# LambdaLabsML/distributed-training-guide

Measured on NVIDIA H100. Metric: tokens/sec (device-timed, max over ranks) Llama-2-7B seq 4096 bf16 training, higher is better.
Workload: dtype bf16; 1 GPU; model=meta-llama/Llama-2-7b-hf, global_batch=1, seq_len=4096, parallelism=dp1 (ddp+zero1), optimizer=AdamW, bf16 parameters and states

## Files before the change

distributed_training_guide_b200/csrc/gemm_common.cuh:

```cuda
#pragma once
#include <cuda.h>
#include <cuda_bf16.h>
#include <cstdint>

#include "common.cuh"

#ifndef DTG_DEFAULT_GEMM_VARIANT
#define DTG_DEFAULT_GEMM_VARIANT 3
#endif

namespace dtg {

template <int CG>
struct GemmCfg {
  static constexpr int THREADS = 384;
  static constexpr int BM = 128;
  static constexpr int BN = 256;
  static constexpr int BK = 64;
  static constexpr int B_ROWS = BN / CG;
  static constexpr int A_BYTES = BM * BK * 2;
  static constexpr int B_BYTES = BN * BK * 2;
  static constexpr int STAGE_BYTES = A_BYTES + B_BYTES;
  static constexpr int STAGES = 4;
  static constexpr int BAR_BYTES = 256;
  static constexpr int SMEM_BYTES = STAGES * STAGE_BYTES + BAR_BYTES + 1024;
  static constexpr int COMM_PIECE = 32768;
  static constexpr int COMM_SLOTS = STAGES * STAGE_BYTES / COMM_PIECE;
  static constexpr int GATHER_PIECE = 16384;
  static constexpr int GATHER_BYTES = 2 * GATHER_PIECE;
  static_assert(2 * STAGES + (COMM_SLOTS > 2 ? COMM_SLOTS : 2) <= BAR_BYTES / 8, "barrier area");
};

template <int N>
struct TmapSet {
  CUtensorMap m[N];
};

struct GemmDist {
  int rows_per_peer;
  int m_tile_shift;
  int k_shift;
  __nv_bfloat16* c_ptr[kMaxRanks];
  const char* ag_src[kMaxRanks];
  uint32_t* ag_flags;
  uint32_t ag_epoch;
  uint32_t* pads[kMaxRanks];
  uint32_t bar_epoch;
  int n_comm;
  int rank, nranks;
  long long tile_bytes;
  const char* bg_src[kMaxRanks];
  char* bg_dst;
  long long bg_per_bytes;
  long long bg_begin, bg_end;
  uint32_t* bg_cnt;
  uint32_t bg_target;
  int bg_chunk_shift;
  int bg_row_bytes;
  int bg_rows;
  int n_tile_shift;
  int group_m, num_n_tiles;
};

#ifdef __CUDACC__
__host__ __device__ __forceinline__ int tile_m(int t, int num_m_tiles, const GemmDist& d) {
  int m = t % num_m_tiles + d.m_tile_shift;
  return m >= num_m_tiles ? m - num_m_tiles : m;
}
__host__ __device__ __forceinline__ void tile_mn(int t, int num_m_tiles, const GemmDist& d, int local_m_tiles, int& m, int& n) {
  if (local_m_tiles <= 0) {
    if (d.group_m > 0 && d.group_m < num_m_tiles) {
      const int per_group = d.group_m * d.num_n_tiles;
      const int g = t / per_group, r = t - g * per_group;
      const int m0 = g * d.group_m;
      const int rest_m = num_m_tiles - m0;
      const int gsz = d.group_m < rest_m ? d.group_m : rest_m;
      m = m0 + r % gsz;
      n = r / gsz;
      return;
    }
    m = tile_m(t, num_m_tiles, d);
    n = t / num_m_tiles + d.n_tile_shift;
    if (n >= d.num_n_tiles && d.n_tile_shift) n -= d.num_n_tiles;
    return;
  }
  const int num_n = d.k_shift;
  const int phase_a = local_m_tiles * num_n;
  int mm;
  if (t < phase_a) {
    mm = t % local_m_tiles;
    n = t / local_m_tiles;
  } else {
    const int u = t - phase_a, rest = num_m_tiles - local_m_tiles;
    mm = local_m_tiles + u % rest;
    n = u / rest;
  }
  mm += d.m_tile_shift;
  m = mm >= num_m_tiles ? mm - num_m_tiles : mm;
}
#endif

CUtensorMap make_tmap_bf16(const void* base, int rank, const uint64_t* dims, const uint64_t* strides_bytes,
                           const uint32_t* box, bool swizzle128);
CUtensorMap make_tmap_2d(const void* base, uint64_t inner, uint64_t outer, uint64_t row_stride_bytes,
                         uint32_t box_inner, uint32_t box_outer);
void set_gemm_variant(int v);
int default_gemm_variant();

}
```

distributed_training_guide_b200/csrc/gemm_wgmma.cu:

```cuda
#include <cuda.h>
#include <cudaTypedefs.h>

#include <cstdlib>
#include <mutex>
#include <unordered_map>

#include "api.h"
#include "common.cuh"
#include "gemm_common.cuh"
#include "ptx.cuh"

namespace dtg {

using namespace ptx;

__device__ __forceinline__ long long bg_clamp(const GemmDist& d, long long x) {
  return x < d.bg_begin ? d.bg_begin : (x > d.bg_end ? d.bg_end : x);
}
__device__ __forceinline__ int bg_rotation_chunks(const GemmDist& d) {
  return (int)((bg_clamp(d, (long long)(d.rank + 1) * d.bg_per_bytes) - d.bg_begin) >> d.bg_chunk_shift);
}

template <bool A_K, bool B_K, int CG, int A_MODE = 0, int B_MODE = 0, int C_MODE = 0, int ET = 0>
__global__ void __launch_bounds__(GemmCfg<CG>::THREADS, 1)
gemm_bf16_kernel(const __grid_constant__ TmapSet<(A_MODE ? kMaxRanks : 1)> tmAs,
                 const __grid_constant__ TmapSet<(B_MODE ? kMaxRanks : 1)> tmBs, const __grid_constant__ GemmDist dist,
                 __nv_bfloat16* __restrict__ C, int M, int N, int K, long long ldc, int accumulate, int num_m_tiles,
                 int num_tiles, const float* __restrict__ scale_a, const float* __restrict__ scale_b) {
  static_assert(ET == 0 || (A_K && B_K && A_MODE == 0 && B_MODE == 0 && C_MODE == 0),
                "the fp8 GEMM takes K-major operands from one tensor map each");
  using Cfg = GemmCfg<CG>;
  constexpr int BK = ET ? 2 * Cfg::BK : Cfg::BK;
  extern __shared__ uint8_t smem_raw[];
  uint8_t* smem = reinterpret_cast<uint8_t*>((reinterpret_cast<uintptr_t>(smem_raw) + 1023) & ~uintptr_t(1023));
  uint64_t* bars = reinterpret_cast<uint64_t*>(smem + Cfg::STAGES * Cfg::STAGE_BYTES);
  uint64_t* full = bars;
  uint64_t* empty = bars + Cfg::STAGES;
  uint64_t* comm_bar = bars + 2 * Cfg::STAGES;

  const int warp = threadIdx.x >> 5;
  const int lane = threadIdx.x & 31;
  const uint32_t cta_rank = (CG == 2) ? cluster_ctarank() : 0u;
  const int n_comm = (A_MODE == 3) ? dist.n_comm : 0;
  const bool is_comm = (A_MODE == 3) && (int)(blockIdx.x / CG) < n_comm;
  const int cluster_id = (int)(blockIdx.x / CG) - n_comm;
  const int num_clusters = (int)(gridDim.x / CG) - n_comm;
  const int num_kb = (K + BK - 1) / BK;
  const int local_m_tiles = (A_MODE == 3) ? dist.rows_per_peer / (Cfg::BM * CG) : 0;

  if (threadIdx.x == 0) {
    prefetch_tensormap(&tmAs.m[0]);
    prefetch_tensormap(&tmBs.m[0]);
    for (int i = 0; i < Cfg::STAGES; ++i) {
      mbar_init(&full[i], 1);
      mbar_init(&empty[i], 2 * CG);
    }
    if constexpr (A_MODE == 3)
      for (int i = 0; i < Cfg::COMM_SLOTS; ++i) mbar_init(&comm_bar[i], 1);
    if constexpr (B_MODE == 3)
      for (int i = 0; i < 2; ++i) mbar_init(&comm_bar[i], 1);
    fence_barrier_init();
  }
  if (CG == 2) cluster_sync(); else __syncthreads();

  if (is_comm) {
    if (warp == 0 && elect_one()) {
      const int cidx = (int)blockIdx.x;
      const int ncta = n_comm * CG;
      const int t_ = dist.nranks, rk = dist.rank;
      for (int p = 0; p < t_; ++p) st_release_sys(dist.pads[p] + cidx * kMaxRanks + rk, dist.bar_epoch);
      for (int p = 0; p < t_; ++p) {
        const uint32_t* mine = dist.pads[rk] + cidx * kMaxRanks + p;
        const unsigned long long t0 = global_timer_ns();
        while ((int32_t)(ld_acquire_sys(mine) - dist.bar_epoch) < 0)
          if (global_timer_ns() - t0 > kWaitTimeoutNs)
            __trap();
      }
      constexpr uint32_t PIECE = Cfg::COMM_PIECE;
      constexpr int NB = Cfg::COMM_SLOTS, AHEAD = NB - 2;
      const int lmt = local_m_tiles > 0 ? local_m_tiles : 1;
      const int remote_tiles = (t_ - 1) * lmt;
      const uint32_t pieces_per_tile = (uint32_t)(dist.tile_bytes / PIECE);
      uint32_t issued = 0, stored = 0;
      for (int r = cidx; r < remote_tiles; r += ncta) {
        const int k = 1 + r / lmt, within = r % lmt;
        const int owner = (rk + k) % t_;
        const int m_tile = owner * lmt + within;
        const char* src = dist.ag_src[k] + (long long)m_tile * dist.tile_bytes;
        char* dst = const_cast<char*>(dist.ag_src[0]) + (long long)m_tile * dist.tile_bytes;
        uint32_t li = 0;
        for (uint32_t si = 0; si < pieces_per_tile; ++si) {
          while (li < pieces_per_tile && li < si + AHEAD) {
            const uint32_t slot = issued % NB;
            bulk_wait_group_read<1>();
            mbar_arrive_expect_tx(&comm_bar[slot], PIECE);
            bulk_load_g2s(smem + slot * PIECE, src + (long long)li * PIECE, PIECE, &comm_bar[slot]);
            ++issued;
            ++li;
          }
          const uint32_t slot = stored % NB;
          mbar_wait_mma(&comm_bar[slot], (stored / NB) & 1);
          bulk_store_s2g(dst + (long long)si * PIECE, smem + slot * PIECE, PIECE);
          bulk_commit_group();
          ++stored;
        }
        bulk_wait_group<0>();
        fence_proxy_async_all();
        st_release_gpu(dist.ag_flags + m_tile, dist.ag_epoch);
      }
    }
  } else if (warp == 0) {
    if (elect_one()) {
      int stage = 0;
      uint32_t phase = 0;
      [[maybe_unused]] int bg_wm = 0;
      [[maybe_unused]] const int bg_nch = (B_MODE == 3) ? (int)((dist.bg_end - dist.bg_begin) >> dist.bg_chunk_shift) : 0;
      [[maybe_unused]] const int bg_rot = (B_MODE == 3) ? bg_rotation_chunks(dist) : 0;
      [[maybe_unused]] const int bg_my0 = (B_MODE == 3)
          ? (int)((bg_clamp(dist, (long long)dist.rank * dist.bg_per_bytes) - dist.bg_begin) >> dist.bg_chunk_shift) : 0;
      [[maybe_unused]] const int bg_tail = bg_nch - bg_rot;
      [[maybe_unused]] auto bg_wait_rows = [&](int r0, int r1) {
        if (r1 > dist.bg_rows) r1 = dist.bg_rows;
        if (r0 >= r1) return;
        const int c0 = (int)(((long long)r0 * dist.bg_row_bytes) >> dist.bg_chunk_shift);
        const int c1 = (int)((((long long)r1 * dist.bg_row_bytes) - 1) >> dist.bg_chunk_shift);
        int need = 0;
        for (int c = c0; c <= c1; ++c) {
          if (c >= bg_my0 && c < bg_rot) continue;
          const int ci = c >= bg_rot ? c - bg_rot : bg_tail + c;
          need = ci + 1 > need ? ci + 1 : need;
        }
        if (need <= bg_wm) return;
        const uint32_t* cnt = dist.bg_cnt + (dist.bg_begin >> dist.bg_chunk_shift);
        while (bg_wm < need) {
          const int c = bg_wm < bg_tail ? bg_rot + bg_wm : bg_wm - bg_tail;
// ... 71 lines not shown
                tma_load_2d_mc(&tmB, &full[stage], sb + (cta_rank * (Cfg::B_ROWS / 64) + j) * 8192, nb + 64 * j, b_k0,
                               0b11);
            }
          }
          if (++stage == Cfg::STAGES) { stage = 0; phase ^= 1; }
        }
      }
    }
  } else if (warp == 1 && !is_comm) {
    if constexpr (B_MODE == 3) {
      if (elect_one()) {
        constexpr uint32_t PIECE = Cfg::GATHER_PIECE;
        uint8_t* gs = smem + Cfg::STAGES * Cfg::STAGE_BYTES + Cfg::BAR_BYTES;
        const int ch = (int)blockIdx.x, nr = dist.nranks, rk = dist.rank;
        for (int p = 0; p < nr && dist.bar_epoch; ++p)
          st_release_sys(dist.pads[p] + ch * kMaxRanks + rk, dist.bar_epoch);
        for (int p = 0; p < nr && dist.bar_epoch; ++p) {
          const uint32_t* mine = dist.pads[rk] + ch * kMaxRanks + p;
          const unsigned long long t0 = global_timer_ns();
          while ((int32_t)(ld_acquire_sys(mine) - dist.bar_epoch) < 0)
            if (global_timer_ns() - t0 > kWaitTimeoutNs)
              __trap();
        }
        static_assert(PIECE == (1u << 14), "16 KB pieces");
        const long long my_lo = bg_clamp(dist, (long long)rk * dist.bg_per_bytes);
        const long long my_hi = bg_clamp(dist, (long long)(rk + 1) * dist.bg_per_bytes);
        const long long total = (dist.bg_end - dist.bg_begin) / PIECE;
        const long long mine = (my_hi - my_lo) / PIECE;
        const long long np = total - mine;
        const long long after = (dist.bg_end - my_hi) / PIECE;
        uint32_t* const cnt = dist.bg_cnt;
        auto flat_of = [&](long long i) {
          return i < after ? my_hi + i * (long long)PIECE : dist.bg_begin + (i - after) * (long long)PIECE;
        };
        auto issue = [&](long long i, uint32_t it) {
          const long long flat = flat_of(i);
          const int owner = (int)(flat / dist.bg_per_bytes);
          const char* src = dist.bg_src[owner] + (flat - (long long)owner * dist.bg_per_bytes);
          const uint32_t slot = it & 1;
          mbar_arrive_expect_tx(&comm_bar[slot], PIECE);
          bulk_load_g2s(gs + slot * PIECE, src, PIECE, &comm_bar[slot]);
        };
        const long long first = blockIdx.x, stride = gridDim.x;
        uint32_t it = 0;
        long long prev_flat = -1;
        if (first < np) issue(first, 0);
        for (long long i = first; i < np; i += stride, ++it) {
          if (i + stride < np) {
            bulk_wait_group_read<0>();
            issue(i + stride, it + 1);
          }
          const uint32_t slot = it & 1;
          mbar_wait_mma(&comm_bar[slot], (it >> 1) & 1);
          const long long flat = flat_of(i);
          bulk_store_s2g(dist.bg_dst + flat, gs + slot * PIECE, PIECE);
          bulk_commit_group();
          if (prev_flat >= 0) {
            bulk_wait_group<1>();
            fence_proxy_async_all();
            red_release_gpu_add(cnt + (prev_flat >> dist.bg_chunk_shift), 1u);
          }
          prev_flat = flat;
        }
        if (prev_flat >= 0) {
          bulk_wait_group<0>();
          fence_proxy_async_all();
          red_release_gpu_add(cnt + (prev_flat >> dist.bg_chunk_shift), 1u);
        }
      }
    }
  } else if (warp >= 4 && !is_comm) {
    const int half = (warp >> 2) - 1;
    const int wq = warp & 3;
    const bool signal = (threadIdx.x & 127) == 0;
    const uint32_t peer_empty = (CG == 2) ? mapa(smem_u32(&empty[0]), cta_rank ^ 1u) : 0u;
    auto release = [&](int s) {
      if (signal) {
        mbar_arrive(&empty[s]);
        if constexpr (CG == 2) mbar_arrive_cluster(peer_empty + (uint32_t)(s * 8));
      }
    };
    int stage = 0;
    uint32_t phase = 0;
    for (int t = cluster_id; t < num_tiles; t += num_clusters) {
      int tm_, tn_;
      tile_mn(t, num_m_tiles, dist, local_m_tiles, tm_, tn_);
      const int m0 = tm_ * (Cfg::BM * CG) + (int)cta_rank * Cfg::BM + half * 64;
      const int n0 = tn_ * Cfg::BN;
      float acc[128];
#pragma unroll
      for (int i = 0; i < 128; ++i) acc[i] = 0.f;
      int prev = -1;
      for (int kb = 0; kb < num_kb; ++kb) {
        mbar_wait_mma(&full[stage], phase);
        const uint32_t a_base = smem_u32(smem + stage * Cfg::STAGE_BYTES) + (uint32_t)(half * 8192);
        const uint32_t b_base = smem_u32(smem + stage * Cfg::STAGE_BYTES + Cfg::A_BYTES);
        wgmma_fence();
        fence_regs(acc);
        if constexpr (ET == 0) {
#pragma unroll
          for (int k = 0; k < Cfg::BK / 16; ++k) {
            const uint64_t da = A_K ? desc_kmajor_sw128(a_base + k * 32) : desc_mnmajor_sw128(a_base + k * 2048, 8192);
            const uint64_t db = B_K ? desc_kmajor_sw128(b_base + k * 32) : desc_mnmajor_sw128(b_base + k * 2048, 8192);
            wgmma_m64n256k16_ss<A_K ? 0 : 1, B_K ? 0 : 1>(acc, da, db, 1u);
          }
        } else {
#pragma unroll
          for (int k = 0; k < BK / 32; ++k)
            wgmma_m64n256k32_fp8_ss<ET>(acc, desc_kmajor_sw128(a_base + k * 32), desc_kmajor_sw128(b_base + k * 32), 1u);
        }
        wgmma_commit();
        wgmma_wait<1>();
        fence_regs(acc);
        if (prev >= 0) release(prev);
        prev = stage;
        if (++stage == Cfg::STAGES) { stage = 0; phase ^= 1; }
      }
      wgmma_wait<0>();
      fence_regs(acc);
      if (prev >= 0) release(prev);
      [[maybe_unused]] float deq = 1.f;
      if constexpr (ET != 0) deq = scale_a[0] * scale_b[0];
      const int r0 = m0 + wq * 16 + (lane >> 2);
      const int c0 = n0 + 2 * (lane & 3);
#pragma unroll
      for (int h = 0; h < 2; ++h) {
        const int row = r0 + 8 * h;
        if (row >= M) continue;
        __nv_bfloat16* crow = C + (size_t)row * ldc;
        if constexpr (C_MODE == 1) {
          const int owner = row / dist.rows_per_peer;
          crow = dist.c_ptr[owner < kMaxRanks ? owner : 0] + (size_t)(row - owner * dist.rows_per_peer) * ldc;
        }
#pragma unroll
        for (int j = 0; j < 32; ++j) {
          const int col = c0 + 8 * j;
          if (col < N) {
            float x = acc[4 * j + 2 * h], y = acc[4 * j + 2 * h + 1];
            if constexpr (ET != 0) {
              x *= deq;
              y *= deq;
            }
            __nv_bfloat162* p = reinterpret_cast<__nv_bfloat162*>(crow + col);
            if (accumulate) {
              const float2 g = __bfloat1622float2(*p);
              x += g.x;
              y += g.y;
            }
            *p = __floats2bfloat162_rn(x, y);
          }
        }
      }
    }
  }

  if (CG == 2) cluster_sync();
}


static PFN_cuTensorMapEncodeTiled_v12000 get_encode_fn() {
  static PFN_cuTensorMapEncodeTiled_v12000 fn = nullptr;
  if (!fn) {
    void* p = nullptr;
    cudaDriverEntryPointQueryResult qres;
    DTG_CUDA_CHECK(cudaGetDriverEntryPoint("cuTensorMapEncodeTiled", &p, cudaEnableDefault, &qres));
    if (qres != cudaDriverEntryPointSuccess || !p) throw std::runtime_error("cuTensorMapEncodeTiled unavailable");
    fn = reinterpret_cast<PFN_cuTensorMapEncodeTiled_v12000>(p);
  }
  return fn;
}

static CUtensorMap make_tmap_typed(CUtensorMapDataType dtype, const void* base, int rank, const uint64_t* dims,
                                   const uint64_t* strides_bytes, const uint32_t* box, bool swizzle128) {
  static thread_local bool ctx_bound = false;
  if (!ctx_bound) {
    int dev = 0;
    DTG_CUDA_CHECK(cudaGetDevice(&dev));
    DTG_CUDA_CHECK(cudaSetDevice(dev));
    DTG_CUDA_CHECK(cudaFree(nullptr));
    ctx_bound = true;
  }
  CUtensorMap m;
  cuuint64_t gdim[5];
  cuuint64_t gstr[4];
  cuuint32_t bdim[5], estr[5];
  for (int i = 0; i < rank; ++i) {
    gdim[i] = dims[i];
    bdim[i] = box[i];
    estr[i] = 1;
    if (i > 0) gstr[i - 1] = strides_bytes[i - 1];
  }
  CUresult r = get_encode_fn()(&m, dtype, (cuuint32_t)rank, const_cast<void*>(base), gdim,
                               gstr, bdim, estr, CU_TENSOR_MAP_INTERLEAVE_NONE,
                               swizzle128 ? CU_TENSOR_MAP_SWIZZLE_128B : CU_TENSOR_MAP_SWIZZLE_NONE,
                               CU_TENSOR_MAP_L2_PROMOTION_L2_256B, CU_TENSOR_MAP_FLOAT_OOB_FILL_NONE);
  if (r != CUDA_SUCCESS) {
    throw std::runtime_error("cuTensorMapEncodeTiled failed with code " + std::to_string((int)r) +
                             " (base must be 16B aligned, strides multiples of 16B)");
  }
  return m;
}

CUtensorMap make_tmap_bf16(const void* base, int rank, const uint64_t* dims, const uint64_t* strides_bytes,
                           const uint32_t* box, bool swizzle128) {
  return make_tmap_typed(CU_TENSOR_MAP_DATA_TYPE_BFLOAT16, base, rank, dims, strides_bytes, box, swizzle128);
}

CUtensorMap make_tmap_2d(const void* base, uint64_t inner, uint64_t outer, uint64_t row_stride_bytes, uint32_t box_inner,
                         uint32_t box_outer) {
  uint64_t dims[2] = {inner, outer};
  uint64_t strides[1] = {row_stride_bytes};
  uint32_t box[2] = {box_inner, box_outer};
  return make_tmap_bf16(base, 2, dims, strides, box, true);
}

static CUtensorMap make_tmap_2d_u8(const void* base, uint64_t inner, uint64_t outer, uint64_t row_stride_bytes,
                                   uint32_t box_inner, uint32_t box_outer) {
  uint64_t dims[2] = {inner, outer};
  uint64_t strides[1] = {row_stride_bytes};
  uint32_t box[2] = {box_inner, box_outer};
  return make_tmap_typed(CU_TENSOR_MAP_DATA_TYPE_UINT8, base, 2, dims, strides, box, true);
}

static int g_gemm_variant = 0;
void set_gemm_variant(int v) { g_gemm_variant = v; }
int default_gemm_variant() {
  if (g_gemm_variant) return g_gemm_variant;
  static int env = -1;
  if (env < 0) {
    const char* e = getenv("DTG_GEMM_VARIANT");
    env = e ? atoi(e) : DTG_DEFAULT_GEMM_VARIANT;
  }
  return env;
}

template <bool A_K, bool B_K, int CG, int A_MODE, int B_MODE, int C_MODE, int ET = 0>
static void launch_gemm(const void* const* a_srcs, const void* const* b_srcs, void* C, int M, int N, int K,
                        long long lda, long long ldb, long long ldc, bool accumulate, GemmDist dist, int nranks,
                        cudaStream_t s, const float* scale_a = nullptr, const float* scale_b = nullptr) {
  using Cfg = GemmCfg<CG>;
  constexpr int ESIZE = ET ? 1 : 2;
  TmapSet<(A_MODE ? kMaxRanks : 1)> tmA;
  TmapSet<(B_MODE ? kMaxRanks : 1)> tmB;
  const int rpp = dist.rows_per_peer;
  for (int p = 0; p < ((A_MODE == 1 || A_MODE == 2) ? nranks : 1); ++p) {
    const int rows = (A_MODE == 1) ? rpp : M;
    const int ks = (A_MODE == 2) ? rpp : K;
    if constexpr (ET != 0) tmA.m[p] = make_tmap_2d_u8(a_srcs[p], ks, rows, lda, 128, Cfg::BM);
    else tmA.m[p] = A_K ? make_tmap_2d(a_srcs[p], ks, rows, lda * 2, 64, Cfg::BM) : make_tmap_2d(a_srcs[p], rows, ks, lda * 2, 64, 64);
  }
  for (int p = 0; p < ((B_MODE == 1 || B_MODE == 2) ? nranks : 1); ++p) {
    const int ks = (B_MODE == 2) ? rpp : K;
    if constexpr (ET != 0) tmB.m[p] = make_tmap_2d_u8(b_srcs[p], ks, N, ldb, 128, Cfg::B_ROWS);
    else tmB.m[p] = B_K ? make_tmap_2d(b_srcs[p], ks, N, ldb * 2, 64, Cfg::B_ROWS) : make_tmap_2d(b_srcs[p], N, ks, ldb * 2, 64, 64);
  }
  for (int p = ((A_MODE == 1 || A_MODE == 2) ? nranks : 1); p < (A_MODE ? kMaxRanks : 1); ++p) tmA.m[p] = tmA.m[0];
  for (int p = ((B_MODE == 1 || B_MODE == 2) ? nranks : 1); p < (B_MODE ? kMaxRanks : 1); ++p) tmB.m[p] = tmB.m[0];
  const int num_m_tiles = (M + Cfg::BM * CG - 1) / (Cfg::BM * CG);
  const int num_n_tiles = (N + Cfg::BN - 1) / Cfg::BN;
  const int num_tiles = num_m_tiles * num_n_tiles;
  auto kern = gemm_bf16_kernel<A_K, B_K, CG, A_MODE, B_MODE, C_MODE, ET>;
  constexpr int kSmem = Cfg::SMEM_BYTES + (B_MODE == 3 ? Cfg::GATHER_BYTES : 0);
  static bool attr_set = false;
  if (!attr_set) {
    DTG_CUDA_CHECK(cudaFuncSetAttribute(kern, cudaFuncAttributeMaxDynamicSharedMemorySize, kSmem));
    attr_set = true;
  }
  dist.num_n_tiles = num_n_tiles;
  if constexpr (A_MODE == 0 && B_MODE == 0 && C_MODE == 0) {
    static const long long budget = []() {
      const char* e = getenv("DTG_GEMM_L2_BUDGET_MB");
      return (long long)(e ? atoi(e) : 16) << 20;
    }();
    const long long panel = (long long)Cfg::BM * CG * K * ESIZE;
    long long gm = budget / (panel > 0 ? panel : 1);
    if (gm < 8) gm = 8;
    dist.group_m = gm >= num_m_tiles ? 0 : (int)gm;
  }
  int clusters = sm_count() / CG;
  if constexpr (A_MODE == 3) {
    dist.k_shift = num_n_tiles;
    int gemm_clusters = clusters - dist.n_comm;
    if (gemm_clusters > num_tiles) gemm_clusters = num_tiles;
    clusters = gemm_clusters + dist.n_comm;
  } else if (clusters > num_tiles) {
    clusters = num_tiles;
  }
  cudaLaunchConfig_t cfg{};
  cfg.gridDim = dim3(clusters * CG);
  cfg.blockDim = dim3(Cfg::THREADS);
  cfg.dynamicSmemBytes = kSmem;
  cfg.stream = s;
  cudaLaunchAttribute attrs[1];
  attrs[0].id = cudaLaunchAttributeClusterDimension;
  attrs[0].val.clusterDim.x = CG;
  attrs[0].val.clusterDim.y = 1;
  attrs[0].val.clusterDim.z = 1;
  cfg.attrs = attrs;
  cfg.numAttrs = 1;
  DTG_CUDA_CHECK(cudaLaunchKernelEx(&cfg, kern, tmA, tmB, dist, (__nv_bfloat16*)C, M, N, K, ldc, accumulate ? 1 : 0,
                                    num_m_tiles, num_tiles, scale_a, scale_b));
  note_launch();
}

int gemm_max_active_clusters(int cg) {
  cudaLaunchConfig_t cfg{};
  cfg.blockDim = dim3(GemmCfg<1>::THREADS);
  cudaLaunchAttribute attrs[1];
  attrs[0].id = cudaLaunchAttributeClusterDimension;
  attrs[0].val.clusterDim.x = cg;
  attrs[0].val.clusterDim.y = 1;
  attrs[0].val.clusterDim.z = 1;
  cfg.attrs = attrs;
  cfg.numAttrs = 1;
  int n = -1;
  if (cg == 2) {
    auto kern = gemm_bf16_kernel<true, true, 2, 0, 0, 0>;
    cfg.gridDim = dim3(sm_count());
    cfg.dynamicSmemBytes = GemmCfg<2>::SMEM_BYTES;
    cudaFuncSetAttribute(kern, cudaFuncAttributeMaxDynamicSharedMemorySize, GemmCfg<2>::SMEM_BYTES);
    cudaOccupancyMaxActiveClusters(&n, kern, &cfg);
  } else {
    auto kern = gemm_bf16_kernel<true, true, 1, 0, 0, 0>;
    cfg.gridDim = dim3(sm_count());
    cfg.dynamicSmemBytes = GemmCfg<1>::SMEM_BYTES;
    cudaFuncSetAttribute(kern, cudaFuncAttributeMaxDynamicSharedMemorySize, GemmCfg<1>::SMEM_BYTES);
    cudaOccupancyMaxActiveClusters(&n, kern, &cfg);
  }
  return n;
}

static void check_gemm_bases(const char* who, const void* A, const void* B, const void* C) {
  const struct { const void* p; const char* name; } ops[3] = {{A, "A"}, {B, "B"}, {C, "C"}};
  for (const auto& o : ops)
    if (reinterpret_cast<uintptr_t>(o.p) % 16)
      throw std::runtime_error(std::string(who) + ": " + o.name + " must start at a 16-byte aligned address");
}

static void gemm_empty_k(void* C, int M, int N, long long ldc, bool accumulate, cudaStream_t s) {
  if (!accumulate)
    DTG_CUDA_CHECK(cudaMemset2DAsync(C, (size_t)ldc * 2, 0, (size_t)N * 2, (size_t)M, s));
}

void gemm_bf16(const void* A, const void* B, void* C, int M, int N, int K, long long lda, long long ldb, long long ldc,
               bool a_kmajor, bool b_kmajor, bool accumulate, int variant, cudaStream_t s) {
  if (M <= 0 || N <= 0) return;
  if ((N % 8) || (ldc % 8) || (lda % 8) || (ldb % 8))
    throw std::runtime_error("gemm_bf16: N and the leading dimensions must be multiples of 8 elements");
  check_gemm_bases("gemm_bf16", A, B, C);
  if (K <= 0) return gemm_empty_k(C, M, N, ldc, accumulate, s);
  if (variant == 0) variant = default_gemm_variant();
  if (variant == 3) variant = (M > 128) ? 2 : 1;
  const int cg = (variant == 2) ? 2 : 1;
  const void* as[1] = {A};
  const void* bs[1] = {B};
  GemmDist dist{};
#define DTG_GEMM_CASE(AK, BK)                                                                                    \
  if (a_kmajor == AK && b_kmajor == BK) {                                                                        \
    if (cg == 2) launch_gemm<AK, BK, 2, 0, 0, 0>(as, bs, C, M, N, K, lda, ldb, ldc, accumulate, dist, 1, s);      \
    else launch_gemm<AK, BK, 1, 0, 0, 0>(as, bs, C, M, N, K, lda, ldb, ldc, accumulate, dist, 1, s);              \
    return;                                                                                                      \
  }
  DTG_GEMM_CASE(true, true)
  DTG_GEMM_CASE(true, false)
  DTG_GEMM_CASE(false, false)
  DTG_GEMM_CASE(false, true)
#undef DTG_GEMM_CASE
}

void gemm_fp8(const void* A, const void* B, void* C, int M, int N, int K, long long lda, long long ldb, long long ldc,
              bool a_e5m2, const float* scale_a, const float* scale_b, bool accumulate, int variant, cudaStream_t s) {
  if (M <= 0 || N <= 0) return;
  if ((N % 16) || (lda % 16) || (ldb % 16) || (ldc % 16))
    throw std::runtime_error("gemm_fp8: N and the leading dimensions must be multiples of 16 elements (TMA needs "
                             "16-byte row strides of the fp8 operands)");
  check_gemm_bases("gemm_fp8", A, B, C);
  if (K <= 0) return gemm_empty_k(C, M, N, ldc, accumulate, s);
  if (variant == 0) variant = default_gemm_variant();
  if (variant == 3) variant = (M > 128) ? 2 : 1;
  const int cg = (variant == 2) ? 2 : 1;
  const void* as[1] = {A};
  const void* bs[1] = {B};
  GemmDist dist{};
#define DTG_GEMM_FP8_CASE(ET)                                                                                     \
  if (cg == 2) launch_gemm<true, true, 2, 0, 0, 0, ET>(as, bs, C, M, N, K, lda, ldb, ldc, accumulate, dist, 1, s,  \
                                                       scale_a, scale_b);                                        \
  else launch_gemm<true, true, 1, 0, 0, 0, ET>(as, bs, C, M, N, K, lda, ldb, ldc, accumulate, dist, 1, s, scale_a, \
                                               scale_b);
  if (a_e5m2) {
    DTG_GEMM_FP8_CASE(2)
  } else {
    DTG_GEMM_FP8_CASE(1)
  }
#undef DTG_GEMM_FP8_CASE
}

void gemm_bf16_dist(int mode, const void* const* a_srcs, const void* const* b_srcs, void* const* c_dsts, int M, int N,
                    int K, long long lda, long long ldb, long long ldc, bool b_kmajor, bool accumulate, int nranks,
                    int rank, int rows_per_peer, cudaStream_t s) {
  if ((N % 8) || (ldc % 8) || (lda % 8) || (ldb % 8))
    throw std::runtime_error("gemm_bf16_dist: N and the leading dimensions must be multiples of 8 elements");
  if (nranks < 1 || nranks > kMaxRanks) throw std::runtime_error("gemm_bf16_dist: 1..8 ranks");
  GemmDist dist{};
  dist.rows_per_peer = rows_per_peer;
  constexpr int TM = GemmCfg<2>::BM * 2;
  if (mode == 1 || mode == 2) {
    if (rows_per_peer % TM != 0 || rows_per_peer * nranks != M)
      throw std::runtime_error("gemm_bf16_dist: rows per rank must be a multiple of 256 and sum to M");
    dist.m_tile_shift = (mode == 1) ? rank * (rows_per_peer / TM) : ((rank + 1) % nranks) * (rows_per_peer / TM);
// ... 99 lines not shown
```

distributed_training_guide_b200/csrc/ptx.cuh:

```cuda
#pragma once
#include <cuda.h>
#include <cuda_bf16.h>
#include <cstdint>
#include <cstdio>

namespace dtg {
namespace ptx {

__device__ __forceinline__ uint32_t smem_u32(const void* p) { return (uint32_t)__cvta_generic_to_shared(p); }

__device__ __forceinline__ uint32_t lane_id() {
  uint32_t l;
  asm volatile("mov.u32 %0, %%laneid;" : "=r"(l));
  return l;
}

__device__ __forceinline__ bool elect_one() {
  uint32_t pred = 0;
  asm volatile(
      "{\n\t"
      ".reg .pred P1;\n\t"
      "elect.sync _|P1, 0xffffffff;\n\t"
      "selp.u32 %0, 1, 0, P1;\n\t"
      "}\n"
// ... 2 lines not shown
}

__device__ __forceinline__ uint32_t cluster_ctarank() {
  uint32_t r;
  asm volatile("mov.u32 %0, %%cluster_ctarank;" : "=r"(r));
  return r;
}
__device__ __forceinline__ void cluster_arrive() { asm volatile("barrier.cluster.arrive.release.aligned;" ::: "memory"); }
__device__ __forceinline__ void cluster_wait() { asm volatile("barrier.cluster.wait.acquire.aligned;" ::: "memory"); }
__device__ __forceinline__ void cluster_sync() {
  cluster_arrive();
  cluster_wait();
}
__device__ __forceinline__ uint32_t mapa(uint32_t smem_addr, uint32_t rank) {
  uint32_t r;
  asm volatile("mapa.shared::cluster.u32 %0, %1, %2;" : "=r"(r) : "r"(smem_addr), "r"(rank));
  return r;
}

__device__ __forceinline__ void mbar_init(uint64_t* bar, uint32_t count) {
  asm volatile("mbarrier.init.shared::cta.b64 [%0], %1;" ::"r"(smem_u32(bar)), "r"(count));
}
__device__ __forceinline__ void fence_barrier_init() { asm volatile("fence.mbarrier_init.release.cluster;" ::: "memory"); }
__device__ __forceinline__ void fence_proxy_async() { asm volatile("fence.proxy.async.shared::cta;" ::: "memory"); }

__device__ __forceinline__ void mbar_arrive(uint64_t* bar) {
  asm volatile("mbarrier.arrive.shared::cta.b64 _, [%0];" ::"r"(smem_u32(bar)) : "memory");
}
__device__ __forceinline__ void mbar_arrive_cluster(uint32_t cluster_addr) {
  asm volatile("mbarrier.arrive.shared::cluster.b64 _, [%0];" ::"r"(cluster_addr) : "memory");
}
__device__ __forceinline__ void mbar_arrive_expect_tx(uint64_t* bar, uint32_t bytes) {
  asm volatile("mbarrier.arrive.expect_tx.shared::cta.b64 _, [%0], %1;" ::"r"(smem_u32(bar)), "r"(bytes) : "memory");
}
__device__ __forceinline__ bool mbar_try_wait(uint64_t* bar, uint32_t parity) {
  uint32_t ok;
  asm volatile(
      "{\n\t"
      ".reg .pred p;\n\t"
      "mbarrier.try_wait.parity.shared::cta.b64 p, [%1], %2;\n\t"
      "selp.u32 %0, 1, 0, p;\n\t"
      "}\n"
      : "=r"(ok)
      : "r"(smem_u32(bar)), "r"(parity)
      : "memory");
  return ok != 0;
}
__device__ __forceinline__ unsigned long long global_timer_ns() {
  unsigned long long t;
  asm volatile("mov.u64 %0, %%globaltimer;" : "=l"(t));
  return t;
}
constexpr unsigned long long kWaitTimeoutNs = 8ULL * 1000 * 1000 * 1000;
static __device__ __noinline__ void wait_timeout_trap(const char* what, const char* file, unsigned line) {
  printf("[dtg] %s:%u: %s — block (%d,%d,%d) thread %d; trapping\n", file, line, what, (int)blockIdx.x, (int)blockIdx.y,
         (int)blockIdx.z, (int)threadIdx.x);
  __threadfence_system();
  __trap();
}
__device__ __forceinline__ void mbar_wait_at(uint64_t* bar, uint32_t parity, const char* file, unsigned line) {
  if (mbar_try_wait(bar, parity)) return;
  uint32_t polls = 0;
  unsigned long long t0 = 0;
  while (!mbar_try_wait(bar, parity)) {
    if ((++polls & 0xFFFFu) == 0) {
      const unsigned long long now = global_timer_ns();
      if (t0 == 0) t0 = now;
      else if (now - t0 > kWaitTimeoutNs) wait_timeout_trap("mbarrier wait timed out (pipeline deadlock)", file, line);
    }
  }
}
#define mbar_wait(bar, parity) ::dtg::ptx::mbar_wait_at((bar), (parity), __FILE__, __LINE__)
__device__ __forceinline__ void mbar_wait_mma(uint64_t* bar, uint32_t parity) {
  if (mbar_try_wait(bar, parity)) return;
  uint32_t polls = 0;
  unsigned long long t0 = 0;
  while (!mbar_try_wait(bar, parity)) {
    if ((++polls & 0xFFFFu) == 0) {
      const unsigned long long now = global_timer_ns();
      if (t0 == 0) t0 = now;
      else if (now - t0 > kWaitTimeoutNs) __trap();
    }
  }
}

__device__ __forceinline__ void named_bar_sync(int id, int nthreads) {
  asm volatile("bar.sync %0, %1;" ::"r"(id), "r"(nthreads) : "memory");
}
__device__ __forceinline__ float fast_exp2(float x) {
  float y;
  asm("ex2.approx.ftz.f32 %0, %1;" : "=f"(y) : "f"(x));
  return y;
}

__device__ __forceinline__ float poly_exp2(float x) {
  x = fmaxf(x, -126.f);
  float t;
  asm("add.rm.ftz.f32 %0, %1, %2;" : "=f"(t) : "f"(x), "f"(12582912.f));
  const float f = x - (t - 12582912.f);
  float p = fmaf(0.077119089663028717f, f, 0.227564394474029541f);
  p = fmaf(p, f, 0.695146143436431885f);
  p = fmaf(p, f, 1.0f);
  return __int_as_float(__float_as_int(p) + (__float_as_int(t) << 23));
}

__device__ __forceinline__ void prefetch_tensormap(const CUtensorMap* m) {
  asm volatile("prefetch.tensormap [%0];" ::"l"(reinterpret_cast<uint64_t>(m)) : "memory");
}
__device__ __forceinline__ void tma_load_2d(const CUtensorMap* m, uint64_t* bar, void* smem, int c0, int c1) {
  asm volatile(
      "cp.async.bulk.tensor.2d.shared::cluster.global.mbarrier::complete_tx::bytes [%0], [%1, {%3, %4}], [%2];"
      :
      : "r"(smem_u32(smem)), "l"(reinterpret_cast<uint64_t>(m)), "r"(smem_u32(bar)), "r"(c0), "r"(c1)
      : "memory");
}
__device__ __forceinline__ void tma_load_2d_mc(const CUtensorMap* m, uint64_t* bar, void* smem, int c0, int c1,
                                               uint16_t cta_mask) {
  asm volatile(
      "cp.async.bulk.tensor.2d.shared::cluster.global.mbarrier::complete_tx::bytes.multicast::cluster [%0], [%1, {%3, %4}], "
      "[%2], %5;"
      :
      : "r"(smem_u32(smem)), "l"(reinterpret_cast<uint64_t>(m)), "r"(smem_u32(bar)), "r"(c0), "r"(c1), "h"(cta_mask)
      : "memory");
}
__device__ __forceinline__ void tma_load_3d(const CUtensorMap* m, uint64_t* bar, void* smem, int c0, int c1, int c2) {
  asm volatile(
      "cp.async.bulk.tensor.3d.shared::cluster.global.mbarrier::complete_tx::bytes [%0], [%1, {%3, %4, %5}], [%2];"
      :
      : "r"(smem_u32(smem)), "l"(reinterpret_cast<uint64_t>(m)), "r"(smem_u32(bar)), "r"(c0), "r"(c1), "r"(c2)
      : "memory");
}
__device__ __forceinline__ void tma_load_4d(const CUtensorMap* m, uint64_t* bar, void* smem, int c0, int c1, int c2,
                                            int c3) {
  asm volatile(
      "cp.async.bulk.tensor.4d.shared::cluster.global.mbarrier::complete_tx::bytes [%0], [%1, {%3, %4, %5, %6}], [%2];"
      :
      : "r"(smem_u32(smem)), "l"(reinterpret_cast<uint64_t>(m)), "r"(smem_u32(bar)), "r"(c0), "r"(c1), "r"(c2),
        "r"(c3)
      : "memory");
}
__device__ __forceinline__ void tma_store_2d(const CUtensorMap* m, const void* smem, int c0, int c1) {
  asm volatile("cp.async.bulk.tensor.2d.global.shared::cta.bulk_group [%0, {%2, %3}], [%1];"
               :
               : "l"(reinterpret_cast<uint64_t>(m)), "r"(smem_u32(smem)), "r"(c0), "r"(c1)
               : "memory");
}
__device__ __forceinline__ void tma_store_4d(const CUtensorMap* m, const void* smem, int c0, int c1, int c2, int c3) {
  asm volatile("cp.async.bulk.tensor.4d.global.shared::cta.bulk_group [%0, {%2, %3, %4, %5}], [%1];"
               :
               : "l"(reinterpret_cast<uint64_t>(m)), "r"(smem_u32(smem)), "r"(c0), "r"(c1), "r"(c2), "r"(c3)
               : "memory");
}
__device__ __forceinline__ void tma_store_commit() { asm volatile("cp.async.bulk.commit_group;" ::: "memory"); }
template <int N>
__device__ __forceinline__ void tma_store_wait_read() {
  asm volatile("cp.async.bulk.wait_group.read %0;" ::"n"(N) : "memory");
}
template <int N>
__device__ __forceinline__ void tma_store_wait() {
  asm volatile("cp.async.bulk.wait_group %0;" ::"n"(N) : "memory");
}

__device__ __forceinline__ void bulk_load_g2s(void* smem, const void* gsrc, uint32_t bytes, uint64_t* bar) {
  asm volatile("cp.async.bulk.shared::cluster.global.mbarrier::complete_tx::bytes [%0], [%1], %2, [%3];"
               :
               : "r"(smem_u32(smem)), "l"(gsrc), "r"(bytes), "r"(smem_u32(bar))
// ... 197 lines not shown
```

Before: 8790 tokens/s.

## Stage GEMM epilogue through shared memory and write C with TMA stores

Adds a TMA-based epilogue for the WGMMA GEMM: each consumer warpgroup writes its bf16 results into a swizzled shared-memory staging buffer and issues 64x64 TMA box stores, instead of scattered per-thread global stores. For accumulate mode, the existing C tile is prefetched with TMA loads before the mainloop and added in shared memory. This is meant to make C writes and reads coalesced and asynchronous. In exchange it needs extra shared memory, named barriers and store-wait synchronization, and it only applies when B_MODE!=3 and C_MODE==0.

```diff
diff --git a/distributed_training_guide_b200/csrc/gemm_common.cuh b/distributed_training_guide_b200/csrc/gemm_common.cuh
--- a/distributed_training_guide_b200/csrc/gemm_common.cuh
+++ b/distributed_training_guide_b200/csrc/gemm_common.cuh
@@ -28,7 +28,14 @@
   static constexpr int COMM_SLOTS = STAGES * STAGE_BYTES / COMM_PIECE;
   static constexpr int GATHER_PIECE = 16384;
   static constexpr int GATHER_BYTES = 2 * GATHER_PIECE;
-  static_assert(2 * STAGES + (COMM_SLOTS > 2 ? COMM_SLOTS : 2) <= BAR_BYTES / 8, "barrier area");
+  static constexpr int EPI_BOX_BYTES = 64 * 64 * 2;
+  static constexpr int EPI_WG_BYTES = 2 * EPI_BOX_BYTES;
+  static constexpr int EPI_OFFSET = STAGES * STAGE_BYTES + 1024;
+  static constexpr int SMEM_BYTES_EPI = EPI_OFFSET + 2 * EPI_WG_BYTES + 1024;
+  static constexpr int EPI_BAR = 2 * STAGES + 8;
+  static_assert(2 * STAGES + (COMM_SLOTS > 2 ? COMM_SLOTS : 2) <= EPI_BAR && EPI_BAR + 2 <= BAR_BYTES / 8,
+                "barrier area");
+  static_assert(SMEM_BYTES_EPI <= 232448, "staging buffer exceeds the 227 KB of shared memory a CTA may have");
 };
 
 template <int N>
diff --git a/distributed_training_guide_b200/csrc/gemm_wgmma.cu b/distributed_training_guide_b200/csrc/gemm_wgmma.cu
--- a/distributed_training_guide_b200/csrc/gemm_wgmma.cu
+++ b/distributed_training_guide_b200/csrc/gemm_wgmma.cu
@@ -14,6 +14,8 @@
 
 using namespace ptx;
 
+template <int B_MODE, int C_MODE>
+constexpr bool kTmaEpilogue = (B_MODE != 3 && C_MODE == 0);
 __device__ __forceinline__ long long bg_clamp(const GemmDist& d, long long x) {
   return x < d.bg_begin ? d.bg_begin : (x > d.bg_end ? d.bg_end : x);
 }
@@ -25,11 +27,13 @@
 __global__ void __launch_bounds__(GemmCfg<CG>::THREADS, 1)
 gemm_bf16_kernel(const __grid_constant__ TmapSet<(A_MODE ? kMaxRanks : 1)> tmAs,
                  const __grid_constant__ TmapSet<(B_MODE ? kMaxRanks : 1)> tmBs, const __grid_constant__ GemmDist dist,
-                 __nv_bfloat16* __restrict__ C, int M, int N, int K, long long ldc, int accumulate, int num_m_tiles,
-                 int num_tiles, const float* __restrict__ scale_a, const float* __restrict__ scale_b) {
+                 const __grid_constant__ CUtensorMap tmC, __nv_bfloat16* __restrict__ C, int M, int N, int K,
+                 long long ldc, int accumulate, int num_m_tiles, int num_tiles, const float* __restrict__ scale_a,
+                 const float* __restrict__ scale_b) {
   static_assert(ET == 0 || (A_K && B_K && A_MODE == 0 && B_MODE == 0 && C_MODE == 0),
                 "the fp8 GEMM takes K-major operands from one tensor map each");
   using Cfg = GemmCfg<CG>;
+  constexpr bool TMA_EPI = kTmaEpilogue<B_MODE, C_MODE>;
   constexpr int BK = ET ? 2 * Cfg::BK : Cfg::BK;
   extern __shared__ uint8_t smem_raw[];
   uint8_t* smem = reinterpret_cast<uint8_t*>((reinterpret_cast<uintptr_t>(smem_raw) + 1023) & ~uintptr_t(1023));
@@ -51,6 +55,10 @@
   if (threadIdx.x == 0) {
     prefetch_tensormap(&tmAs.m[0]);
     prefetch_tensormap(&tmBs.m[0]);
+    if constexpr (TMA_EPI) {
+      prefetch_tensormap(&tmC);
+      for (int i = 0; i < 2; ++i) mbar_init(&bars[Cfg::EPI_BAR + i], 1);
+    }
     for (int i = 0; i < Cfg::STAGES; ++i) {
       mbar_init(&full[i], 1);
       mbar_init(&empty[i], 2 * CG);
@@ -288,11 +296,24 @@
     };
     int stage = 0;
     uint32_t phase = 0;
+    [[maybe_unused]] uint8_t* const stg = smem + Cfg::EPI_OFFSET + half * Cfg::EPI_WG_BYTES;
+    [[maybe_unused]] uint64_t* const c_bar = bars + Cfg::EPI_BAR + half;
+    [[maybe_unused]] uint32_t c_phase = 0;
+    [[maybe_unused]] const uint32_t stg_s = smem_u32(stg) + (uint32_t)((wq * 16 + (lane >> 2)) * 128 + 4 * (lane & 3));
+    [[maybe_unused]] const int bar_id = 1 + half;
     for (int t = cluster_id; t < num_tiles; t += num_clusters) {
       int tm_, tn_;
       tile_mn(t, num_m_tiles, dist, local_m_tiles, tm_, tn_);
       const int m0 = tm_ * (Cfg::BM * CG) + (int)cta_rank * Cfg::BM + half * 64;
       const int n0 = tn_ * Cfg::BN;
+      if constexpr (TMA_EPI) {
+        if (accumulate && signal && m0 < M) {
+          const int nbox = n0 + 64 < N ? 2 : 1;
+          tma_store_wait_read<0>();
+          mbar_arrive_expect_tx(c_bar, nbox * Cfg::EPI_BOX_BYTES);
+          for (int b = 0; b < nbox; ++b) tma_load_2d(&tmC, c_bar, stg + b * Cfg::EPI_BOX_BYTES, n0 + 64 * b, m0);
+        }
+      }
       float acc[128];
 #pragma unroll
       for (int i = 0; i < 128; ++i) acc[i] = 0.f;
@@ -327,6 +348,61 @@
       if (prev >= 0) release(prev);
       [[maybe_unused]] float deq = 1.f;
       if constexpr (ET != 0) deq = scale_a[0] * scale_b[0];
+      if constexpr (TMA_EPI) {
+        if (m0 >= M) continue;
+#pragma unroll
+        for (int p = 0; p < 2; ++p) {
+          const int c0 = n0 + 128 * p;
+          if (c0 >= N) break;
+          const int nbox = c0 + 64 < N ? 2 : 1;
+          if (accumulate) {
+            if (p == 1 && signal) {
+              tma_store_wait_read<0>();
+              mbar_arrive_expect_tx(c_bar, nbox * Cfg::EPI_BOX_BYTES);
+              for (int b = 0; b < nbox; ++b) tma_load_2d(&tmC, c_bar, stg + b * Cfg::EPI_BOX_BYTES, c0 + 64 * b, m0);
+            }
+            mbar_wait_mma(c_bar, c_phase);
+            c_phase ^= 1;
+          } else {
+            if (signal) tma_store_wait_read<0>();
+            named_bar_sync(bar_id, 128);
+          }
+#pragma unroll
+          for (int b = 0; b < 2; ++b) {
+#pragma unroll
+            for (int jj = 0; jj < 8; ++jj) {
+              const int j = 16 * p + 8 * b + jj;
+#pragma unroll
+              for (int h = 0; h < 2; ++h) {
+                float x = acc[4 * j + 2 * h], y = acc[4 * j + 2 * h + 1];
+                const uint32_t q = stg_s + (uint32_t)(b * Cfg::EPI_BOX_BYTES + h * 1024 + ((jj ^ (lane >> 2)) << 4));
+                if (accumulate) {
+                  const uint32_t old = ld_shared_u32(q);
+                  const float2 g = __bfloat1622float2(*reinterpret_cast<const __nv_bfloat162*>(&old));
+                  if constexpr (ET != 0) {
+                    x = __fmaf_rn(x, deq, g.x);
+                    y = __fmaf_rn(y, deq, g.y);
+                  } else {
+                    x += g.x;
+                    y += g.y;
+                  }
+                } else if constexpr (ET != 0) {
+                  x = __fmul_rn(x, deq);
+                  y = __fmul_rn(y, deq);
+                }
+                st_shared_u32(q, pack_bf16x2(x, y));
+              }
+            }
+          }
+          fence_proxy_async();
+          named_bar_sync(bar_id, 128);
+          if (signal) {
+            for (int b = 0; b < nbox; ++b) tma_store_2d(&tmC, stg + b * Cfg::EPI_BOX_BYTES, c0 + 64 * b, m0);
+            tma_store_commit();
+          }
+        }
+        continue;
+      }
       const int r0 = m0 + wq * 16 + (lane >> 2);
       const int c0 = n0 + 2 * (lane & 3);
 #pragma unroll
@@ -358,6 +434,8 @@
         }
       }
     }
+    if constexpr (TMA_EPI)
+      if (signal) tma_store_wait<0>();
   }
 
   if (CG == 2) cluster_sync();
@@ -465,8 +543,11 @@
   const int num_m_tiles = (M + Cfg::BM * CG - 1) / (Cfg::BM * CG);
   const int num_n_tiles = (N + Cfg::BN - 1) / Cfg::BN;
   const int num_tiles = num_m_tiles * num_n_tiles;
+  CUtensorMap tmC{};
+  if constexpr (kTmaEpilogue<B_MODE, C_MODE>) tmC = make_tmap_2d(C, N, M, ldc * 2, 64, 64);
   auto kern = gemm_bf16_kernel<A_K, B_K, CG, A_MODE, B_MODE, C_MODE, ET>;
-  constexpr int kSmem = Cfg::SMEM_BYTES + (B_MODE == 3 ? Cfg::GATHER_BYTES : 0);
+  constexpr int kSmem = kTmaEpilogue<B_MODE, C_MODE> ? Cfg::SMEM_BYTES_EPI
+                                                     : Cfg::SMEM_BYTES + (B_MODE == 3 ? Cfg::GATHER_BYTES : 0);
   static bool attr_set = false;
   if (!attr_set) {
     DTG_CUDA_CHECK(cudaFuncSetAttribute(kern, cudaFuncAttributeMaxDynamicSharedMemorySize, kSmem));
@@ -504,8 +585,8 @@
   attrs[0].val.clusterDim.z = 1;
   cfg.attrs = attrs;
   cfg.numAttrs = 1;
-  DTG_CUDA_CHECK(cudaLaunchKernelEx(&cfg, kern, tmA, tmB, dist, (__nv_bfloat16*)C, M, N, K, ldc, accumulate ? 1 : 0,
-                                    num_m_tiles, num_tiles, scale_a, scale_b));
+  DTG_CUDA_CHECK(cudaLaunchKernelEx(&cfg, kern, tmA, tmB, dist, tmC, (__nv_bfloat16*)C, M, N, K, ldc,
+                                    accumulate ? 1 : 0, num_m_tiles, num_tiles, scale_a, scale_b));
   note_launch();
 }
 
@@ -523,14 +604,14 @@
   if (cg == 2) {
     auto kern = gemm_bf16_kernel<true, true, 2, 0, 0, 0>;
     cfg.gridDim = dim3(sm_count());
-    cfg.dynamicSmemBytes = GemmCfg<2>::SMEM_BYTES;
-    cudaFuncSetAttribute(kern, cudaFuncAttributeMaxDynamicSharedMemorySize, GemmCfg<2>::SMEM_BYTES);
+    cfg.dynamicSmemBytes = GemmCfg<2>::SMEM_BYTES_EPI;
+    cudaFuncSetAttribute(kern, cudaFuncAttributeMaxDynamicSharedMemorySize, GemmCfg<2>::SMEM_BYTES_EPI);
     cudaOccupancyMaxActiveClusters(&n, kern, &cfg);
   } else {
     auto kern = gemm_bf16_kernel<true, true, 1, 0, 0, 0>;
     cfg.gridDim = dim3(sm_count());
-    cfg.dynamicSmemBytes = GemmCfg<1>::SMEM_BYTES;
-    cudaFuncSetAttribute(kern, cudaFuncAttributeMaxDynamicSharedMemorySize, GemmCfg<1>::SMEM_BYTES);
+    cfg.dynamicSmemBytes = GemmCfg<1>::SMEM_BYTES_EPI;
+    cudaFuncSetAttribute(kern, cudaFuncAttributeMaxDynamicSharedMemorySize, GemmCfg<1>::SMEM_BYTES_EPI);
     cudaOccupancyMaxActiveClusters(&n, kern, &cfg);
   }
   return n;
diff --git a/distributed_training_guide_b200/csrc/ptx.cuh b/distributed_training_guide_b200/csrc/ptx.cuh
--- a/distributed_training_guide_b200/csrc/ptx.cuh
+++ b/distributed_training_guide_b200/csrc/ptx.cuh
@@ -108,6 +108,15 @@
       else if (now - t0 > kWaitTimeoutNs) __trap();
     }
   }
+}
+
+__device__ __forceinline__ void st_shared_u32(uint32_t addr, uint32_t v) {
+  asm volatile("st.shared.b32 [%0], %1;" ::"r"(addr), "r"(v) : "memory");
+}
+__device__ __forceinline__ uint32_t ld_shared_u32(uint32_t addr) {
+  uint32_t v;
+  asm volatile("ld.shared.b32 %0, [%1];" : "=r"(v) : "r"(addr) : "memory");
+  return v;
 }
 
 __device__ __forceinline__ void named_bar_sync(int id, int nthreads) {
```

Result: faster. 9097 tokens/s, median of 6 (+3.5%).
